# JackShDr/InfluentialRS

Measured on AMD Instinct MI355X. Metric: scored user-item pairs/sec (whole node), higher is better.
Workload: dtype f32; 1 GPU; c2: n_item=3415, d=128, L=200, H=4, layers=6, ffn=256; one greedy path-search step; users_per_gpu=4096, top_k=100, sweep=bf16 filter + exact f32 re-score, parallelism=single GPU

## Files before the change

### influentialrs_amd/csrc/irs_internal.h

```cpp
#pragma once

#include <hip/hip_runtime.h>
#include <stdint.h>
#include <stdio.h>
#include <string.h>

#include "../../include/irs_hip.h"

#if !defined(IRS_LAB) && (defined(X6_DUMP) || defined(X6_STAMP) || defined(X6_NO_SPLIT) || defined(X6_NO_MFMA) ||            \
                          defined(X6_NO_READS) || defined(X6_NO_DMA) || defined(X6_NO_BARRIER) || defined(X6_NO_QKV_STORE) ||  \
                          defined(X6_NW) || defined(SEQ_EXP) || defined(PLAN_STAMP) || defined(ATTN_STAMP) ||                  \
                          defined(IRS_SMALL_TIMING) || defined(IRS_DIRECT_TIMING))
#error "a lab switch (X6_* / SEQ_EXP / *_STAMP / IRS_*_TIMING) is defined without IRS_LAB: the product library must be built without them"
#endif

#include <atomic>
#include <functional>
#define IRS_MAX_DEVICES 32
static inline int irs_cur_dev() {
    int d = 0;
    if (hipGetDevice(&d) != hipSuccess || d < 0 || d >= IRS_MAX_DEVICES) d = 0;
    return d;
}
#define IRS_ONCE_PER_DEVICE(body_)                                                                                        \
    do {                                                                                                                  \
        static std::atomic<unsigned> once_mask_{0};                                                                       \
        const unsigned once_bit_ = 1u << irs_cur_dev();                                                                   \
        if (!(once_mask_.load(std::memory_order_acquire) & once_bit_)) {                                                  \
            body_;                                                                                                        \
            once_mask_.fetch_or(once_bit_, std::memory_order_release);                                                    \
        }                                                                                                                 \
    } while (0)

#define IRS_MAX_LAYERS 16
#define IRS_CAND_BUCKETS 64
#define IRS_CAND_SLOTS 64
#define IRS_CAND_CAP (IRS_CAND_BUCKETS * IRS_CAND_SLOTS)
#define IRS_REFINE_CAP 1024
#define IRS_MAX_GROUPS 2048
#define IRS_MAX_PATH 64
#define IRS_MAX_EXCL 4096
#define IRS_LSE_SLOTS_RING 4096
#define IRS_COOP_FALLBACK_MIN_ITEMS 262144
#define IRS_EXH_SCRATCH_KEYS (64 * 32768)

struct irs_layer_w {
    const float *sa_in_w, *sa_in_b, *sa_out_w, *sa_out_b;
    const float *ca_in_w, *ca_in_b, *ca_out_w, *ca_out_b;
    const float *l1_w, *l1_b, *l2_w, *l2_b;
    const float *n1_w, *n1_b, *n2_w, *n2_b, *n3_w, *n3_b;
};

struct irs_prof_ev {
    hipEvent_t a, b;
};

enum { IRS_STEP_GREEDY = 1, IRS_STEP_BEAM, IRS_STEP_SHARDED_BEAM, IRS_STEP_SHARDED_BEAM_SPLIT };
struct irs_step_key {
    int32_t kind, B, W, P, k, sweep, sample, sample_k;
    uint64_t seed;
    const void *comm, *seq, *user, *hep, *paths, *status;
    const void *tr_item, *tr_target, *tr_rank, *tr_scratch;
    int32_t arr_rank;
    uint32_t arr_lp_bits;
};
static_assert(sizeof(irs_step_key) == 8 * sizeof(int32_t) + 11 * 8 + 2 * sizeof(int32_t), "irs_step_key is compared with memcmp: no padding");
struct irs_step_graph {
    hipGraphExec_t exec;
    irs_step_key key;
};

struct irs_excl {
    const int64_t *rows;
    const int32_t *cnt;
    const int32_t *map;
    const float *paths;
    const int32_t *step_ptr;
    int stride, div;
    int path_ld, path_by_user;
    int step_arg, on;
};

struct irs_beam_state {
    int64_t *seq;
    int32_t *hep;
    double *cum;
    float *paths;
    int32_t *fin;
};
struct irs_beam_side {
    int64_t *user;
    int32_t *done;
    int32_t *map;
};
struct irs_beam_cand {
    const float *val;
// ... 591 lines not shown
```

### influentialrs_amd/csrc/score.hip

```cpp
#include <type_traits>

#include "irs_internal.h"

typedef __attribute__((ext_vector_type(16))) float f32x16;
typedef __attribute__((ext_vector_type(8))) __bf16 bf16x8;

#define MODE_PRE 0
#define MODE_EMIT 1
#define MODE_COUNT 2
#define MODE_DENSE 3
#define MODE_LSE 4
#define MODE_CEGRAD 5
#define MODE_TRACE 6

struct SweepArgs {
    const uint4 *wp;
    const float *w32;
    const float *bias;
    const uint4 *xb;
    const float *x32;
    int M, M_pad, UT, d;
    int64_t n_local;
    int tile_begin, tile_end, tiles_per_wave, n_strips, n_ublocks;
    int tile_stride;
// ... 1333 lines not shown
    int row = blockIdx.x * 4 + (threadIdx.x >> 6);
    int lane = threadIdx.x & 63;
    if (fb_count && blockIdx.x == 0 && threadIdx.x == 0) *fb_count = 0u;
    if (row >= M_pad) return;
    cand_cnt[(size_t)row * IRS_CAND_BUCKETS + lane] = 0u;
    if (lane == 0 && row < M) status[row] = 0;
    const int ut = row >> 5, r = row & 31;
    float ss = 0.f, ssr = 0.f, ssd = 0.f;
    if (lane < 2 * KS) {
        uint4 v = pack8_bf16(x + (size_t)row * d, 8 * lane, d, row < M, ss, ssr, ssd);
        xb[((size_t)ut * KS + (lane >> 1)) * 64 + (lane & 1) * 32 + r] = v;
    }
    ss = lanes_sum<63>(ss);
    ssr = lanes_sum<63>(ssr);
    ssd = lanes_sum<63>(ssd);
    if (lane == 0) {
        const float nx = sqrtf(fmaxf(ss, ssr)), ndx = sqrtf(ssd);
        const float e = (row < M) ? 1.001f * (ndx * wn[0] + nx * wn[1]) + acc_factor * (1.001f * nx * wn[0] + wn[2]) : 0.f;
        eps[row] = e;
        if (thr_carry && row < M) {
            float t = thr_carry[row];
            if (!(t == t)) t = -INFINITY, thr_carry[row] = t;
            traw_carry[row] = t > -INFINITY ? t + 2.0f * e : -INFINITY;
        }
    }
}

__global__ void k_zero_eps(float *eps, int n) {
    int i = blockIdx.x * blockDim.x + threadIdx.x;
    if (i < n) eps[i] = 0.f;
}

__global__ void __launch_bounds__(256) k_pack_w(const float *__restrict__ W, const float *__restrict__ b, int64_t n_local,
                                                int n_tiles, int d, int KS, uint4 *__restrict__ wp,
                                                float *__restrict__ bias_pad, unsigned int *__restrict__ wn_bits) {
    int64_t row = (int64_t)blockIdx.x * 4 + (threadIdx.x >> 6);
    int lane = threadIdx.x & 63;
    if (row >= (int64_t)n_tiles * 32) return;
    const int64_t t = row >> 5;
    const int r = (int)(row & 31);
    float ss = 0.f, ssr = 0.f, ssd = 0.f;
    if (lane < 2 * KS) {
        uint4 v = pack8_bf16(W + (size_t)row * d, 8 * lane, d, row < n_local, ss, ssr, ssd);
        wp[((size_t)t * KS + (lane >> 1)) * 64 + (lane & 1) * 32 + r] = v;
    }
    ss = lanes_sum<63>(ss);
    ssr = lanes_sum<63>(ssr);
    ssd = lanes_sum<63>(ssd);
    if (lane == 0) {
        bias_pad[row] = (row < n_local) ? b[row] : -INFINITY;
        if (row < n_local) {
            atomicMax(wn_bits + 0, __float_as_uint(sqrtf(fmaxf(ss, ssr)) * 1.001f));
            atomicMax(wn_bits + 1, __float_as_uint(sqrtf(ssd) * 1.001f));
            atomicMax(wn_bits + 2, __float_as_uint(fabsf(b[row])));
        }
    }
}

#define SEL2_G IRS_MAX_GROUPS
static_assert(SEL2_G == 2048, "k_select_thr_bits: 32 keys per lane");
template <int CTRL>
__device__ __forceinline__ unsigned int dpp_u32(unsigned int v) {
    return (unsigned int)__builtin_amdgcn_update_dpp(0, (int)v, CTRL, 0xF, 0xF, true);
}
__device__ __forceinline__ unsigned int wave_sum_u32(unsigned int v) {
    v += dpp_u32<0xB1>(v);
    v += dpp_u32<0x4E>(v);
    v += dpp_u32<0x141>(v);
    v += dpp_u32<0x140>(v);
    return (unsigned int)__builtin_amdgcn_readlane((int)v, 0) + (unsigned int)__builtin_amdgcn_readlane((int)v, 16) +
           (unsigned int)__builtin_amdgcn_readlane((int)v, 32) + (unsigned int)__builtin_amdgcn_readlane((int)v, 48);
}
__device__ __forceinline__ unsigned int wave_max_u32(unsigned int v) {
    unsigned int o;
    o = dpp_u32<0xB1>(v), v = o > v ? o : v;
    o = dpp_u32<0x4E>(v), v = o > v ? o : v;
    o = dpp_u32<0x141>(v), v = o > v ? o : v;
    o = dpp_u32<0x140>(v), v = o > v ? o : v;
    const unsigned int a = (unsigned int)__builtin_amdgcn_readlane((int)v, 0), b = (unsigned int)__builtin_amdgcn_readlane((int)v, 16);
    const unsigned int c = (unsigned int)__builtin_amdgcn_readlane((int)v, 32), d = (unsigned int)__builtin_amdgcn_readlane((int)v, 48);
    const unsigned int ab = a > b ? a : b, cd = c > d ? c : d;
    return ab > cd ? ab : cd;
}
__global__ void __launch_bounds__(256) k_select_thr_bits(const float *__restrict__ gm, int G, int M, int M_pad, int k,
                                                         const float *__restrict__ eps, float *__restrict__ thr,
                                                         float *__restrict__ traw) {
    constexpr int STRIDE = SEL2_G + 16;
    constexpr int KPL = SEL2_G / 64;
    __shared__ unsigned int sel_lds[4 * STRIDE];
    const int tid = threadIdx.x;
    {
        const int rl = tid & 3, tq = tid >> 2;
        const int row = blockIdx.x * 4 + rl;
        const float *blk = gm + (size_t)blockIdx.x * G * 4 + rl;
        float raw[KPL];
#pragma unroll
        for (int i = 0; i < KPL; ++i) {
            const int g = tq + 64 * i;
            raw[i] = blk[(size_t)(g < G ? g : G - 1) * 4];
        }
#pragma unroll
        for (int i = 0; i < KPL; ++i) asm volatile("" : "+v"(raw[i]));
#pragma unroll
        for (int i = 0; i < KPL; ++i) {
            const int g = tq + 64 * i;
            const unsigned int kk = irs_fkey(raw[i]);
            sel_lds[rl * STRIDE + g] = (g < G && row < M) ? kk : 0u;
        }
    }
    __syncthreads();
    const int lane = tid & 63;
    const int wave = __builtin_amdgcn_readfirstlane(tid >> 6);
    const int row = blockIdx.x * 4 + wave;
    unsigned int key[KPL];
    unsigned int mx = 0u, mnc = 0u;
#pragma unroll
    for (int i = 0; i < KPL; ++i) {
        key[i] = sel_lds[wave * STRIDE + lane + 64 * i];
        mx = key[i] > mx ? key[i] : mx;
        const unsigned int c = (lane + 64 * i < G) ? ~key[i] : 0u;
        mnc = c > mnc ? c : mnc;
    }
    const unsigned int smx = wave_max_u32(mx), smn = ~wave_max_u32(mnc);
    const unsigned int diff = smx ^ smn;
    const int top = diff ? 31 - __builtin_clz(diff) : -1;
    unsigned int prefix = top >= 31 ? 0u : (smx & ~((2u << top) - 1u));
    if (top < 0) prefix = smx;
    for (int bit = top; bit >= 0; --bit) {
        const unsigned int cand = prefix | (1u << bit);
        unsigned int c0 = 0, c1 = 0, c2 = 0, c3 = 0;
#pragma unroll
        for (int i = 0; i < KPL; i += 4) {
            c0 += key[i] >= cand ? 1u : 0u;
            c1 += key[i + 1] >= cand ? 1u : 0u;
            c2 += key[i + 2] >= cand ? 1u : 0u;
            c3 += key[i + 3] >= cand ? 1u : 0u;
        }
        const unsigned int cnt = wave_sum_u32((c0 + c1) + (c2 + c3));
        if (cnt >= (unsigned int)k) prefix = cand;
    }
    if (lane == 0 && row < M_pad) {
        const bool enough = G >= k;
        const float t = enough ? irs_unkey(prefix) : -INFINITY;
        thr[row] = (row < M) ? (enough ? t - 2.0f * eps[row] : -INFINITY) : INFINITY;
        traw[row] = (row < M) ? t : INFINITY;
    }
}

__device__ __forceinline__ void bitonic_desc(unsigned long long *keys, int n) {
    for (int size = 2; size <= n; size <<= 1) {
        for (int stride = size >> 1; stride > 0; stride >>= 1) {
            __syncthreads();
            for (int i = threadIdx.x; i < n / 2; i += blockDim.x) {
                int lo = 2 * i - (i & (stride - 1));
                int hi = lo + stride;
                bool desc = ((lo & size) == 0);
                unsigned long long a = keys[lo], b = keys[hi];
                if ((a < b) == desc) {
                    keys[lo] = b;
                    keys[hi] = a;
                }
            }
        }
    }
    __syncthreads();
}

__device__ __forceinline__ void radix_find_bin(const unsigned int *hist, unsigned int need, int lane, int shift,
                                               unsigned int *s_prefix, unsigned int *s_k) {
    const unsigned int h0 = hist[4 * lane], h1 = hist[4 * lane + 1], h2 = hist[4 * lane + 2], h3 = hist[4 * lane + 3];
    const unsigned int own = h0 + h1 + h2 + h3;
// ... 70 lines not shown
        if (i < (int)n) {
            unsigned long long kk = buf[i];
            val[(size_t)row * k + i] = irs_unkey((unsigned int)(kk >> 32));
            ids[(size_t)row * k + i] = item_lo + (int64_t)(0xFFFFFFFFu - (unsigned int)kk);
        } else {
            val[(size_t)row * k + i] = -INFINITY;
            ids[(size_t)row * k + i] = -1;
        }
    }
    if (tid == 0 && (int)n < k) status[row] |= IRS_ROW_FEWER_THAN_K;
}

#define EXH_FB_MAX 64
#define EXH_STRIPS 256
#define EXH_KEYS_PER_ROW 32768

template <typename KeyFn>
__device__ __forceinline__ unsigned int exh_select(KeyFn &&keyfn, int64_t j0, int64_t j1, int k, unsigned long long *buf) {
    __shared__ unsigned int s_n;
    __shared__ unsigned long long s_thr;
    const int tid = threadIdx.x;
    __syncthreads();
    if (tid == 0) {
        s_n = 0;
        s_thr = 0ull;
    }
    __syncthreads();
    for (int64_t base = j0; base < j1; base += 256) {
        const int64_t j = base + tid;
        if (j < j1) {
            const unsigned long long key = keyfn(j);
            if (key > s_thr) {
                const unsigned int slot = atomicAdd(&s_n, 1u);
                buf[slot] = key;
            }
        }
        __syncthreads();
        if (s_n > EXH_BUF - 256) {
            const unsigned int n = s_n;
            for (int i = n + tid; i < EXH_BUF; i += 256) buf[i] = 0ull;
            bitonic_desc(buf, EXH_BUF);
            if (tid == 0) {
                s_n = (n < (unsigned int)k) ? n : k;
                if (n >= (unsigned int)k) s_thr = buf[k - 1];
            }
            __syncthreads();
        }
    }
    const unsigned int n = s_n;
    for (int i = n + tid; i < EXH_BUF; i += 256) buf[i] = 0ull;
    bitonic_desc(buf, EXH_BUF);
    __syncthreads();
    return n < (unsigned int)k ? n : (unsigned int)k;
}

__global__ void __launch_bounds__(256) k_exh_strips(const float *__restrict__ x, int d, const float *__restrict__ W,
                                                    const float *__restrict__ bias, int64_t n_local, int k, int n_strips,
                                                    const unsigned int *__restrict__ fb_count, const int32_t *__restrict__ fb_list,
                                                    unsigned long long *__restrict__ exh_keys) {
    __shared__ unsigned long long buf[EXH_BUF];
    __shared__ float xs[256];
    unsigned int nfb = *fb_count;
    if (nfb == 0u) return;
    if (nfb > EXH_FB_MAX) nfb = EXH_FB_MAX;
    const int strip = blockIdx.x;
    const int64_t per = (n_local + n_strips - 1) / n_strips;
    const int64_t j0 = (int64_t)strip * per, j1 = (j0 + per < n_local) ? j0 + per : n_local;
    for (unsigned int fi = blockIdx.y; fi < nfb; fi += gridDim.y) {
        const int row = fb_list[fi];
        __syncthreads();
        for (int i = threadIdx.x; i < d; i += 256) xs[i] = x[(size_t)row * d + i];
        __syncthreads();
        const unsigned int n = exh_select(
            [&](int64_t j) -> unsigned long long {
                const float e = irs_chain(xs, W + (size_t)j * d, bias[j], d);
                return ((unsigned long long)irs_fkey(e) << 32) | (0xFFFFFFFFu - (unsigned int)j);
            },
            j0, j1, k, buf);
        unsigned long long *o = exh_keys + ((size_t)fi * n_strips + strip) * k;
        for (int i = threadIdx.x; i < k; i += 256) o[i] = i < (int)n ? buf[i] : 0ull;
    }
}

__global__ void __launch_bounds__(256) k_refine(const float *__restrict__ x, int d, const float *__restrict__ W,
                                                const float *__restrict__ bias, const unsigned int *__restrict__ cnt,
                                                const unsigned long long *__restrict__ cand,
                                                const float *__restrict__ eps, const float *__restrict__ traw, int k,
                                                int64_t item_lo, int64_t n_local, float *__restrict__ val,
                                                int64_t *__restrict__ ids, int32_t *__restrict__ status,
                                                unsigned int *__restrict__ fb_count, int32_t *__restrict__ fb_list) {
    __shared__ __attribute__((aligned(16))) unsigned long long ckeys[IRS_CAND_CAP + 2];
    unsigned long long *rkeys = ckeys;
    __shared__ unsigned int hist[256];
    __shared__ float xs[256];
    __shared__ unsigned int boff[IRS_CAND_BUCKETS + 1];
    __shared__ unsigned int s_prefix, s_k, s_nr, s_above, s_over;
    const int row = blockIdx.x, tid = threadIdx.x;
    constexpr int PER = IRS_CAND_BUCKETS * IRS_CAND_SLOTS / 256;
    unsigned long long cv[PER];
#pragma unroll
    for (int j = 0; j < PER; ++j) {
        const int idx = tid + 256 * j;
        cv[j] = cand[((size_t)row * IRS_CAND_BUCKETS + idx / IRS_CAND_SLOTS) * IRS_CAND_SLOTS + idx % IRS_CAND_SLOTS];
    }
    for (int i = tid; i < d; i += 256) xs[i] = x[(size_t)row * d + i];
    if (tid < IRS_CAND_BUCKETS) hist[tid] = cnt[(size_t)row * IRS_CAND_BUCKETS + tid];
    __syncthreads();
    if (tid < 64) {
        const unsigned int cb = hist[tid] & ~IRS_CAND_OVERFLOW;
        const unsigned int cl = cb > IRS_CAND_SLOTS ? IRS_CAND_SLOTS : cb;
        unsigned int incl = cl;
#pragma unroll
        for (int o = 1; o < 64; o <<= 1) {
            const unsigned int t = __shfl_up(incl, o, 64);
            if (tid >= o) incl += t;
        }
        boff[tid] = incl - cl;
        if (tid == 63) boff[IRS_CAND_BUCKETS] = incl;
        const unsigned long long ov = __ballot((hist[tid] & IRS_CAND_OVERFLOW) != 0u);
        if (tid == 0) {
            s_over = ov ? 1u : 0u;
            s_prefix = 0;
            s_k = k;
            s_nr = 0;
            s_above = 0;
        }
    }
    __syncthreads();
    if (s_over) {
        if (tid == 0) status[row] |= IRS_ROW_FALLBACK;
        if (fb_count) {
            if (tid == 0) fb_list[atomicAdd(fb_count, 1u)] = row;
            return;
        }
        exhaustive_row(x, d, W, bias, n_local, item_lo, k, row, val, ids, status, ckeys, xs, true);
        return;
    }
    const unsigned int c = boff[IRS_CAND_BUCKETS];
#pragma unroll
    for (int j = 0; j < PER; ++j) {
        const int idx = tid + 256 * j;
        const int b = idx / IRS_CAND_SLOTS, sl = idx % IRS_CAND_SLOTS;
        if ((unsigned int)sl < boff[b + 1] - boff[b]) ckeys[boff[b] + sl] = cv[j];
    }
    __syncthreads();
    const float t1 = traw[row];
    if (t1 > -INFINITY) {
        unsigned int mine = 0;
        for (int i = tid; i < (int)c; i += 256) mine += (irs_unkey((unsigned int)(ckeys[i] >> 32)) >= t1) ? 1u : 0u;
        if (mine) atomicAdd(&s_above, mine);
        __syncthreads();
        if (s_above < (unsigned int)k) {
            if (tid == 0) status[row] |= IRS_ROW_FALLBACK;
            if (fb_count) {
                if (tid == 0) fb_list[atomicAdd(fb_count, 1u)] = row;
                return;
            }
            exhaustive_row(x, d, W, bias, n_local, item_lo, k, row, val, ids, status, ckeys, xs, false);
            return;
        }
    }
    float thr2 = -INFINITY;
    if (c >= (unsigned int)k) {
        for (int pass = 0; pass < 4; ++pass) {
            const int shift = 24 - 8 * pass;
            hist[tid] = 0;
            __syncthreads();
            const unsigned int prefix = s_prefix;
            for (int i0 = 0; i0 < (int)c; i0 += 256) {
                const int i = i0 + tid;
                const unsigned int key = i < (int)c ? (unsigned int)(ckeys[i] >> 32) : 0u;
                const bool match = i < (int)c && ((pass == 0) || ((key >> (shift + 8)) == (prefix >> (shift + 8))));
                const unsigned int bin = (key >> shift) & 255;
                const unsigned long long m = __ballot(match);
                if (m) {
                    const unsigned int first = __builtin_amdgcn_readlane(bin, __builtin_ctzll(m));
                    if (__ballot(match && bin == first) == m) {
                        if ((tid & 63) == __builtin_ctzll(m)) atomicAdd(&hist[first], (unsigned int)__popcll(m));
                    } else if (match)
                        atomicAdd(&hist[bin], 1u);
                }
            }
            __syncthreads();
            if (tid < 64) radix_find_bin(hist, s_k, tid, shift, &s_prefix, &s_k);
            __syncthreads();
        }
        thr2 = irs_unkey(s_prefix) - 2.0f * eps[row];
    }
    {
        constexpr int PERC = IRS_CAND_CAP / 256;
        unsigned int keep[PERC];
#pragma unroll
        for (int j = 0; j < PERC; ++j) {
            const int i = tid + 256 * j;
            keep[j] = 0xFFFFFFFFu;
            if (i < (int)c) {
                const unsigned long long key = ckeys[i];
                if (irs_unkey((unsigned int)(key >> 32)) >= thr2) keep[j] = (unsigned int)key;
            }
        }
        __syncthreads();
#pragma unroll
        for (int j = 0; j < PERC; ++j)
            if (keep[j] != 0xFFFFFFFFu) rkeys[atomicAdd(&s_nr, 1u)] = (unsigned long long)keep[j];
    }
    __syncthreads();
    const unsigned int nr = s_nr;
    for (int i = tid; i < (int)nr; i += 256) {
        unsigned int j = (unsigned int)rkeys[i];
        float e = irs_chain(xs, W + (size_t)j * d, bias[j], d);
        rkeys[i] = ((unsigned long long)irs_fkey(e) << 32) | (0xFFFFFFFFu - j);
    }
    if ((nr & 1) && tid == 0) rkeys[nr] = 0ull;
    __syncthreads();
    {
        const ulonglong2 *r2 = reinterpret_cast<const ulonglong2 *>(rkeys);
        for (int i = tid; i < (int)nr; i += 256) {
            const unsigned long long me = rkeys[i];
            int above = 0;
            for (int j = 0; j < (int)(nr + 1) / 2; ++j) {
                const ulonglong2 v = r2[j];
                above += (v.x > me) + (v.y > me);
            }
            if (above < k) {
                val[(size_t)row * k + above] = irs_unkey((unsigned int)(me >> 32));
                ids[(size_t)row * k + above] = item_lo + (int64_t)(0xFFFFFFFFu - (unsigned int)me);
            }
        }
        for (int i = (int)nr + tid; i < k; i += 256) {
            val[(size_t)row * k + i] = -INFINITY;
            ids[(size_t)row * k + i] = -1;
        }
    }
    if (tid == 0 && (int)nr < k) status[row] |= IRS_ROW_FEWER_THAN_K;
}

#define DIRECT_MAX_ITEMS 4096
#define DIRECT_TILE 64
#define DIRECT_MAX_D 256
#ifdef IRS_DIRECT_TIMING
__device__ unsigned long long g_direct_t[16];
#define DSTAMP(i) do { if (threadIdx.x == 0) tstamp[i] = __builtin_amdgcn_s_memtime(); } while (0)
#else
#define DSTAMP(i)
#endif
#define DIRECT_ROWS 8
template <int MODE, int SLOTS = IRS_WIN_SLOTS_SHORT>
__global__ void __launch_bounds__(256) k_topk_direct(const float *__restrict__ x, int d, const float *__restrict__ W,
                                                     const float *__restrict__ bias, int n_local, int64_t item_lo, int k,
                                                     unsigned long long *__restrict__ gkeys, unsigned int *__restrict__ arrive,
                                                     float *__restrict__ val, int64_t *__restrict__ ids,
                                                     int32_t *__restrict__ status, irs_path_args pa, int M) {
    __shared__ __attribute__((aligned(16))) float tile[DIRECT_TILE * (DIRECT_MAX_D + 4)];
    __shared__ __attribute__((aligned(16))) unsigned long long rkeys[IRS_REFINE_CAP + 2];
    __shared__ __attribute__((aligned(16))) float xs[(MODE == 1 ? DIRECT_ROWS : 1) * DIRECT_MAX_D];
    __shared__ __attribute__((aligned(16))) unsigned long long tmax[256];
    __shared__ unsigned int wsum[4];
    __shared__ unsigned int s_last, s_thr;
    const int row = MODE == 1 ? blockIdx.y * DIRECT_ROWS : blockIdx.y, tid = threadIdx.x, lane = tid & 63, wave = tid >> 6;
#ifdef IRS_DIRECT_TIMING
    unsigned long long tstamp[10];
#endif
    DSTAMP(0);
    unsigned int *gk = reinterpret_cast<unsigned int *>(gkeys + (size_t)row * IRS_CAND_CAP);
    if constexpr (MODE != 2) {
    const bool vec = (d & 3) == 0;
    const int S = vec ? ((d & 7) ? d : d + 4) : (d | 1);
    const int j0 = blockIdx.x * DIRECT_TILE;
    const int nj = min(DIRECT_TILE, n_local - j0);
    const int d4 = d >> 2;
    if (vec) {
        for (int i = tid; i < nj * d4; i += 256) {
            const int jj = i / d4, c4 = i - jj * d4;
            *reinterpret_cast<float4 *>(tile + jj * S + 4 * c4) = reinterpret_cast<const float4 *>(W + (size_t)j0 * d)[i];
        }
    } else {
        for (int i = tid; i < nj * d; i += 256) {
            const int jj = i / d, c = i - jj * d;
            tile[jj * S + c] = W[(size_t)j0 * d + i];
        }
    }
    if constexpr (MODE == 1) {
        for (int i = tid; i < DIRECT_ROWS * d; i += 256) {
            const int rr = i / d, c = i - rr * d;
            xs[rr * DIRECT_MAX_D + c] = (row + rr < M) ? x[(size_t)(row + rr) * d + c] : 0.f;
        }
        __syncthreads();
        if (lane < nj) {
            const float b0 = bias[j0 + lane];
            float acc0 = b0, acc1 = b0;
            const float *x0 = xs + wave * DIRECT_MAX_D, *x1 = xs + (wave + 4) * DIRECT_MAX_D;
            if (vec) {
                const float4 *w4 = reinterpret_cast<const float4 *>(tile + lane * S);
                for (int c = 0; c < d4; ++c) {
                    const float4 wv = w4[c], xa = reinterpret_cast<const float4 *>(x0)[c], xb = reinterpret_cast<const float4 *>(x1)[c];
                    acc0 = __fmaf_rn(xa.x, wv.x, acc0), acc1 = __fmaf_rn(xb.x, wv.x, acc1);
                    acc0 = __fmaf_rn(xa.y, wv.y, acc0), acc1 = __fmaf_rn(xb.y, wv.y, acc1);
                    acc0 = __fmaf_rn(xa.z, wv.z, acc0), acc1 = __fmaf_rn(xb.z, wv.z, acc1);
                    acc0 = __fmaf_rn(xa.w, wv.w, acc0), acc1 = __fmaf_rn(xb.w, wv.w, acc1);
                }
            } else {
                const float *wr = tile + lane * S;
                for (int c = 0; c < d; ++c) acc0 = __fmaf_rn(x0[c], wr[c], acc0), acc1 = __fmaf_rn(x1[c], wr[c], acc1);
            }
            if (row + wave < M) gk[(size_t)wave * (IRS_CAND_CAP * 2) + j0 + lane] = irs_fkey(acc0);
            if (row + wave + 4 < M) gk[(size_t)(wave + 4) * (IRS_CAND_CAP * 2) + j0 + lane] = irs_fkey(acc1);
        }
        return;
    }
    for (int i = tid; i < d; i += 256) xs[i] = x[(size_t)row * d + i];
    __syncthreads();
    DSTAMP(1);
    if (wave == 0 && lane < nj) {
        float acc = bias[j0 + lane];
        if (vec) {
            const float4 *w4 = reinterpret_cast<const float4 *>(tile + lane * S);
            const float4 *x4 = reinterpret_cast<const float4 *>(xs);
// ... 434 lines not shown
    sweep_decompose(a, 0, ctx->n_tiles, 1, tpw);
    *slots = a.n_strips * 4 * 2;
    if (*slots > 2 * max_waves) IRS_FAIL(ctx, IRS_E_UNSUPPORTED, "lse slots %d > %d", *slots, 2 * max_waves);
    a.lse_part = ctx->lse_part;
    return IRS_OK;
}

static void sweep_f32_whole(const irs_ctx *ctx, SweepArgs &a, const float *xrows, int M) {
    sweep_common(ctx, a, xrows, M);
    const int nub = (a.UT + ub_f32(ctx->KS) - 1) / ub_f32(ctx->KS);
    sweep_decompose(a, 0, ctx->n_tiles, nub, 0);
}

template <bool EMIT>
static int launch_lse_f32(irs_ctx *ctx, SweepArgs &a, hipStream_t s) {
    const int KS = ctx->KS;
    if (lse_ring_ok(ctx, a)) {
        a.n_ublocks = 1;
        constexpr int SPW = LSE_RING_NW / 4;
        const int nwg = (a.n_strips + SPW - 1) / SPW;
        dim3 grid(((nwg + 7) / 8) * 8);
        const size_t lds = (size_t)LSE_RING_NW * LSE_RING_WAVE_B + (size_t)LSE_RING_NW * (EMIT_Q * 12 + 16);
        IRS_ONCE_PER_DEVICE({
            (void)hipFuncSetAttribute(reinterpret_cast<const void *>(k_lse_ring<16, EMIT, LSE_RING_NW, LSE_RING_CK>), hipFuncAttributeMaxDynamicSharedMemorySize, (int)lds);
            (void)hipFuncSetAttribute(reinterpret_cast<const void *>(k_lse_ring<8, EMIT, LSE_RING_NW, LSE_RING_CK>), hipFuncAttributeMaxDynamicSharedMemorySize, (int)lds);
        });
        if (KS == 16) hipLaunchKernelGGL((k_lse_ring<16, EMIT, LSE_RING_NW, LSE_RING_CK>), grid, dim3(64 * LSE_RING_NW), lds, s, a);
        else hipLaunchKernelGGL((k_lse_ring<8, EMIT, LSE_RING_NW, LSE_RING_CK>), grid, dim3(64 * LSE_RING_NW), lds, s, a);
        IRS_CHECK_HIP(ctx, hipGetLastError());
        return IRS_OK;
    }
    const bool xreg = a.UT == 1 && KS == 16;
    const int UB = xreg ? 1 : ub_f32(KS);
    a.n_ublocks = (a.UT + UB - 1) / UB;
    dim3 grid(((a.n_strips + 7) / 8) * 8 * a.n_ublocks);
    const size_t lds = (size_t)UB * KS * 2048 + EMIT_Q_BYTES;
#define L_(KS_, UB_, XR_)                                                                                                 \
    do {                                                                                                                  \
        IRS_ONCE_PER_DEVICE((void)hipFuncSetAttribute(reinterpret_cast<const void *>(k_lse_f32<KS_, UB_, EMIT, XR_>),     \
                                                      hipFuncAttributeMaxDynamicSharedMemorySize, (int)lds));             \
        hipLaunchKernelGGL((k_lse_f32<KS_, UB_, EMIT, XR_>), grid, dim3(256), lds, s, a);                                 \
    } while (0)
    switch (KS) {
    case 2: L_(2, 8, false); break;
    case 4: L_(4, 8, false); break;
    case 8: L_(8, 4, false); break;
    case 16: if (xreg) L_(16, 1, true); else L_(16, 2, false); break;
    default: IRS_FAIL(ctx, IRS_E_UNSUPPORTED, "unsupported d_pad %d", ctx->d_pad);
    }
#undef L_
    IRS_CHECK_HIP(ctx, hipGetLastError());
    return IRS_OK;
}

int irs_launch_pack_w(irs_ctx *ctx, hipStream_t s) {
    IRS_CHECK_HIP(ctx, hipMemsetAsync(ctx->wnorm_max, 0, 4 * sizeof(float), s));
    int64_t rows = (int64_t)ctx->n_tiles * 32;
    hipLaunchKernelGGL(k_pack_w, dim3((unsigned)((rows + 3) / 4)), dim3(256), 0, s, ctx->proj_w, ctx->proj_b,
                       ctx->n_local, ctx->n_tiles, ctx->dims.d, ctx->KS, ctx->wp,
                       ctx->bias_pad, reinterpret_cast<unsigned int *>(ctx->wnorm_max));
    IRS_CHECK_HIP(ctx, hipGetLastError());
    return IRS_OK;
}

bool irs_topk_is_direct(const irs_ctx *ctx, int M, int k) {
    return M <= 1024 && ctx->n_local <= DIRECT_MAX_ITEMS && k <= 256 && ctx->dims.d <= DIRECT_MAX_D;
}

enum TopkForm {
    TOPK_DIRECT1,
    TOPK_DIRECT2,
    TOPK_SWEPT,
};
struct TopkPlan {
    TopkForm form;
    bool fused_lse;
    bool lse_after;
    bool reuse_thr;
    bool coop_fb;
    int stride;
    int nt0;
    int tpw0;
    int r_sel;
};

static TopkPlan topk_plan(const irs_ctx *ctx, const float *xrows, int M, int k, int sweep, bool want_lse, int carry) {
    TopkPlan p{};
    if (irs_topk_is_direct(ctx, M, k)) {
        p.form = M <= 32 ? TOPK_DIRECT1 : TOPK_DIRECT2;
        p.lse_after = want_lse;
        return p;
    }
    p.form = TOPK_SWEPT;
    SweepArgs a;
    sweep_common(ctx, a, xrows, M);
    p.fused_lse = want_lse && sweep == IRS_SWEEP_BF16 && lse_fast_ok(ctx, a);
    p.lse_after = want_lse && !p.fused_lse;
    p.coop_fb = ctx->n_local >= IRS_COOP_FALLBACK_MIN_ITEMS && ctx->exh_keys != nullptr;
    const int nt = ctx->n_tiles;
    p.reuse_thr = carry && ctx->carry_period > 0 && sweep == IRS_SWEEP_BF16 && !p.fused_lse && ctx->thr_valid && ctx->thr_M == M &&
                  ctx->thr_k == k && ctx->thr_age + 1 < ctx->carry_period && nt >= 2 * 8 * 1024;
    if (p.reuse_thr) return p;
    int nt0 = nt >= 16 * 1024 ? nt / 16 : nt / 8;
    if (nt0 < 1024) nt0 = 1024;
    if (nt0 > nt) nt0 = nt;
    p.stride = nt / nt0;
    p.nt0 = (nt + p.stride - 1) / p.stride;
    p.tpw0 = (p.nt0 + 1023) / 1024;
    p.r_sel = k;
    if (p.stride > 1) {
        p.r_sel = ((p.stride >= 16 ? 4 : 3) * k + p.stride - 1) / p.stride;
        if (p.r_sel < 8) p.r_sel = 8;
        if (p.r_sel > k) p.r_sel = k;
    }
    return p;
}

static int topk_direct(irs_ctx *ctx, const TopkPlan &p, const float *xrows, int M, int k, float *val, int64_t *ids0,
                       int32_t *status, const irs_path_args *path, hipStream_t s) {
    irs_prof_begin(ctx, IRS_PROF_REFINE, s);
    const unsigned int tiles = (unsigned)((ctx->n_local + DIRECT_TILE - 1) / DIRECT_TILE);
    unsigned int *arrive = reinterpret_cast<unsigned int *>(ctx->step_ctr) + 8;
    const irs_path_args pa = path ? *path : irs_path_args{};
    constexpr int S16 = IRS_WIN_SLOTS_LONG;
    const bool long_win = path && irs_window_slots(ctx) == S16;
    if (p.form == TOPK_DIRECT1)
        hipLaunchKernelGGL((long_win ? k_topk_direct<0, S16> : k_topk_direct<0>), dim3(tiles, M), dim3(256), 0, s, xrows, ctx->dims.d, ctx->proj_w, ctx->proj_b,
                           (int)ctx->n_local, ctx->shard.item_lo, k, ctx->cand, arrive, val, ids0, status, pa, M);
    else {
        hipLaunchKernelGGL(k_topk_direct<1>, dim3(tiles, (M + DIRECT_ROWS - 1) / DIRECT_ROWS), dim3(256), 0, s, xrows, ctx->dims.d,
                           ctx->proj_w, ctx->proj_b, (int)ctx->n_local, ctx->shard.item_lo, k, ctx->cand, arrive, val, ids0,
                           status, irs_path_args{}, M);
        hipLaunchKernelGGL((long_win ? k_topk_direct<2, S16> : k_topk_direct<2>), dim3(1, M), dim3(256), 0, s, xrows, ctx->dims.d, ctx->proj_w, ctx->proj_b,
                           (int)ctx->n_local, ctx->shard.item_lo, k, ctx->cand, arrive, val, ids0, status, pa, M);
    }
    irs_prof_end(ctx, IRS_PROF_REFINE, s, 2.0 * ctx->dims.d * (double)M * (double)ctx->n_local, 0.0);
    IRS_CHECK_HIP(ctx, hipGetLastError());
    return IRS_OK;
}

static int topk_prep(irs_ctx *ctx, const TopkPlan &p, const float *xrows, int M, int M_pad, int sweep, int32_t *status,
                     hipStream_t s) {
    static_assert(IRS_CAND_BUCKETS == 64, "k_prep_x resets one bucket counter per lane");
    if (sweep == IRS_SWEEP_BF16) {
        const float acc_factor = (float)(ctx->d_pad + 8) * 2.384185791015625e-07f;
        hipLaunchKernelGGL(k_prep_x, dim3((M_pad + 3) / 4), dim3(256), 0, s, xrows, M, M_pad, ctx->dims.d, ctx->KS,
                           ctx->xb, ctx->eps, ctx->wnorm_max, acc_factor, ctx->cand_cnt, status, p.coop_fb ? ctx->fb_count : nullptr,
                           p.reuse_thr ? ctx->thr : nullptr, p.reuse_thr ? ctx->ref_tmp : nullptr);
    } else {
        IRS_CHECK_HIP(ctx, hipMemsetAsync(status, 0, sizeof(int32_t) * M, s));
        IRS_CHECK_HIP(ctx, hipMemsetAsync(ctx->cand_cnt, 0, sizeof(unsigned int) * (size_t)M_pad * IRS_CAND_BUCKETS, s));
        hipLaunchKernelGGL(k_zero_eps, dim3((M_pad + 255) / 256), dim3(256), 0, s, ctx->eps, M_pad);
    }
    IRS_CHECK_HIP(ctx, hipGetLastError());
    return IRS_OK;
}

static int topk_select(irs_ctx *ctx, const TopkPlan &p, SweepArgs &a, int M, int sweep, hipStream_t s) {
    sweep_decompose(a, 0, ctx->n_tiles, 1, p.tpw0, p.stride);
    const int G = 2 * a.n_strips * 4;
    if (G > SEL2_G) IRS_FAIL(ctx, IRS_E_UNSUPPORTED, "pre-pass groups %d > %d", G, SEL2_G);
    a.gm = ctx->gm;
    a.n_groups = G;
    irs_prof_begin(ctx, IRS_PROF_SWEEP, s);
    const int rc = sweep == IRS_SWEEP_BF16 ? launch_sweep_bf16<MODE_PRE>(ctx, a, s) : launch_sweep_f32<MODE_PRE>(ctx, a, s);
    irs_prof_end(ctx, IRS_PROF_SWEEP, s, 2.0 * ctx->dims.d * (double)M * p.nt0 * 32.0,
                 (double)p.nt0 * 32.0 * ctx->d_pad * (sweep == IRS_SWEEP_BF16 ? 2.0 : 4.0));
    if (rc) return rc;
    hipLaunchKernelGGL(k_select_thr_bits, dim3((a.M_pad + 3) / 4), dim3(256), 0, s, ctx->gm, G, M, a.M_pad, p.r_sel, ctx->eps,
                       ctx->thr, ctx->ref_tmp);
    IRS_CHECK_HIP(ctx, hipGetLastError());
    return IRS_OK;
}

static int topk_emit(irs_ctx *ctx, const TopkPlan &p, SweepArgs &a, int M, int sweep, float *lse_max, float *lse_sum,
                     hipStream_t s) {
    a.thr = ctx->thr;
    a.cnt = ctx->cand_cnt;
    a.cand = ctx->cand;
    int lse_slots = 0, rc;
    if (p.fused_lse) {
        if ((rc = lse_decompose(ctx, a, &lse_slots))) return rc;
    } else {
        const int UB = sweep == IRS_SWEEP_BF16 ? ub_bf16(ctx->KS) : ub_f32(ctx->KS);
        sweep_decompose(a, 0, ctx->n_tiles, (a.UT + UB - 1) / UB, 0);
    }
    const double flops = 2.0 * ctx->dims.d * (double)M * (double)ctx->n_local;
    const double bytes = (double)ctx->n_tiles * 32.0 * ctx->d_pad * ((sweep == IRS_SWEEP_BF16 && !p.fused_lse) ? 2.0 : 4.0);
    irs_prof_begin(ctx, IRS_PROF_SWEEP, s);
    irs_prof_begin(ctx, IRS_PROF_SWEEP_EMIT, s);
    if (p.fused_lse) rc = launch_lse_f32<true>(ctx, a, s);
    else if (sweep == IRS_SWEEP_BF16) rc = launch_sweep_bf16<MODE_EMIT>(ctx, a, s);
    else rc = launch_sweep_f32<MODE_EMIT>(ctx, a, s);
    irs_prof_end(ctx, IRS_PROF_SWEEP, s, flops, bytes);
    irs_prof_end(ctx, IRS_PROF_SWEEP_EMIT, s, flops, bytes);
    if (rc) return rc;
    if (p.fused_lse) {
        hipLaunchKernelGGL(k_lse_reduce, dim3(M), dim3(256), 0, s, ctx->lse_part, lse_slots, a.M_pad, M, lse_max, lse_sum);
        IRS_CHECK_HIP(ctx, hipGetLastError());
    }
    return IRS_OK;
}

static int topk_refine(irs_ctx *ctx, const TopkPlan &p, const float *xrows, int M, int k, int sweep, float *val, int64_t *ids0,
                       int32_t *status, hipStream_t s) {
    const int d = ctx->dims.d;
    irs_prof_begin(ctx, IRS_PROF_REFINE, s);
    if (p.coop_fb && sweep != IRS_SWEEP_BF16) IRS_CHECK_HIP(ctx, hipMemsetAsync(ctx->fb_count, 0, sizeof(unsigned int), s));
    hipLaunchKernelGGL(k_refine, dim3(M), dim3(256), 0, s, xrows, d, ctx->proj_w, ctx->proj_b, ctx->cand_cnt, ctx->cand,
                       ctx->eps, ctx->ref_tmp, k, ctx->shard.item_lo, ctx->n_local, val, ids0, status,
                       p.coop_fb ? ctx->fb_count : nullptr, ctx->fb_list);
    if (p.coop_fb) {
        int ns = EXH_STRIPS;
        while (ns > 1 && (long long)ns * k > EXH_KEYS_PER_ROW) ns >>= 1;
        hipLaunchKernelGGL(k_exh_strips, dim3(ns, 4), dim3(256), 0, s, xrows, d, ctx->proj_w, ctx->proj_b, ctx->n_local, k, ns,
                           ctx->fb_count, ctx->fb_list, ctx->exh_keys);
        hipLaunchKernelGGL(k_exh_merge, dim3(EXH_FB_MAX), dim3(256), 0, s, xrows, d, ctx->proj_w, ctx->proj_b, ctx->n_local,
                           ctx->shard.item_lo, k, ns, ctx->fb_count, ctx->fb_list, ctx->exh_keys, val, ids0, status);
    }
    irs_prof_end(ctx, IRS_PROF_REFINE, s, 0.0, 0.0);
    IRS_CHECK_HIP(ctx, hipGetLastError());
    return IRS_OK;
}

int irs_launch_topk(irs_ctx *ctx, const float *xrows, int M, int k, int sweep, float *val, int64_t *ids0,
                    int32_t *status, hipStream_t s, const irs_path_args *path, float *lse_max, float *lse_sum, int carry) {
    const TopkPlan p = topk_plan(ctx, xrows, M, k, sweep, lse_max != nullptr, carry);
    if (path && p.form == TOPK_SWEPT) IRS_FAIL(ctx, IRS_E_STATE, "fused path step needs the direct top-k");
    int rc;
    if (p.form != TOPK_SWEPT) {
        if ((rc = topk_direct(ctx, p, xrows, M, k, val, ids0, status, path, s))) return rc;
    } else {
        SweepArgs a;
        sweep_common(ctx, a, xrows, M);
        if ((rc = topk_prep(ctx, p, xrows, M, a.M_pad, sweep, status, s))) return rc;
        if (p.reuse_thr) ++ctx->thr_age;
        else {
            if ((rc = topk_select(ctx, p, a, M, sweep, s))) return rc;
            ctx->thr_valid = sweep == IRS_SWEEP_BF16, ctx->thr_M = M, ctx->thr_k = k, ctx->thr_age = 0;
        }
        if ((rc = topk_emit(ctx, p, a, M, sweep, lse_max, lse_sum, s))) return rc;
        if ((rc = topk_refine(ctx, p, xrows, M, k, sweep, val, ids0, status, s))) return rc;
    }
    return p.lse_after ? irs_launch_lse(ctx, xrows, M, lse_max, lse_sum, s) : IRS_OK;
}

int irs_launch_topk_exhaustive(irs_ctx *ctx, const float *xrows, int M, int k, float *val, int64_t *ids0,
                               int32_t *status, hipStream_t s) {
    IRS_CHECK_HIP(ctx, hipMemsetAsync(status, 0, sizeof(int32_t) * M, s));
    hipLaunchKernelGGL(k_exhaustive, dim3(M), dim3(256), 0, s, xrows, ctx->dims.d, ctx->proj_w, ctx->proj_b,
                       ctx->n_local, ctx->shard.item_lo, k, 0, val, ids0, status);
    IRS_CHECK_HIP(ctx, hipGetLastError());
    return IRS_OK;
}

int irs_launch_gather(irs_ctx *ctx, const float *xrows, int M, const int64_t *ids0, int g, float *out, hipStream_t s) {
    hipLaunchKernelGGL(k_gather, dim3(M), dim3(64), 0, s, xrows, ctx->dims.d, ctx->proj_w, ctx->proj_b,
                       ctx->shard.item_lo, ctx->n_local, ids0, g, out);
    IRS_CHECK_HIP(ctx, hipGetLastError());
    return IRS_OK;
}

int irs_launch_count_before(irs_ctx *ctx, const float *xrows, int M, const float *ref_score, const int64_t *ref_id0,
                            const int64_t *excl, int n_excl, int64_t *count, hipStream_t s) {
    SweepArgs a;
    sweep_f32_whole(ctx, a, xrows, M);
    IRS_CHECK_HIP(ctx, hipMemsetAsync(count, 0, sizeof(int64_t) * M, s));
    int64_t *ref_local = reinterpret_cast<int64_t *>(ctx->cand);
    hipLaunchKernelGGL(k_localize_ref, dim3((M + 255) / 256), dim3(256), 0, s, ref_id0, ctx->shard.item_lo, ref_local, M);
    a.ref_score = ref_score;
    a.ref_id = ref_local;
    a.count = reinterpret_cast<unsigned long long *>(count);
    irs_prof_begin(ctx, IRS_PROF_SWEEP, s);
    int rc = launch_sweep_f32<MODE_COUNT>(ctx, a, s);
    irs_prof_end(ctx, IRS_PROF_SWEEP, s, 2.0 * ctx->dims.d * (double)M * (double)ctx->n_local,
                 (double)ctx->n_local * ctx->dims.d * 4.0);
    if (rc) return rc;
    if (excl && n_excl > 0) {
        hipLaunchKernelGGL(k_count_excl, dim3(M), dim3(64), 0, s, xrows, ctx->dims.d, ctx->proj_w, ctx->proj_b,
                           ctx->shard.item_lo, ctx->n_local, ref_score, ref_id0, excl, n_excl,
                           reinterpret_cast<unsigned long long *>(count));
    }
    IRS_CHECK_HIP(ctx, hipGetLastError());
    return IRS_OK;
}

int irs_launch_dense(irs_ctx *ctx, const float *xrows, int M, float *out, int64_t ld, hipStream_t s) {
    SweepArgs a;
    sweep_f32_whole(ctx, a, xrows, M);
    a.dense = out;
    a.ld = ld;
    irs_prof_begin(ctx, IRS_PROF_SWEEP, s);
// ... 196 lines not shown
```

Before: 2.394 billion pairs/s.

## Add sparse refine path skipping radix select for small candidate sets; template threshold select

Adds a SPARSE variant of the refine kernel that loads only the occupied candidate slots per bucket via wave-level readlane, computes the bucket prefix in registers instead of through LDS with an extra barrier, and uses a wave-reduced count. When the candidate count is at most 512, it skips the four-pass radix threshold select and re-scores all candidates exactly. The threshold-select kernel is also templated on keys per lane so small group counts use a smaller register and LDS footprint. The trade-off is that small-candidate rows now do more exact f32 dot products in place of the radix passes. Lab-only timestamp instrumentation is added behind a compile switch.

```diff
diff --git a/influentialrs_amd/csrc/irs_internal.h b/influentialrs_amd/csrc/irs_internal.h
--- a/influentialrs_amd/csrc/irs_internal.h
+++ b/influentialrs_amd/csrc/irs_internal.h
@@ -10,8 +10,8 @@
 #if !defined(IRS_LAB) && (defined(X6_DUMP) || defined(X6_STAMP) || defined(X6_NO_SPLIT) || defined(X6_NO_MFMA) ||            \
                           defined(X6_NO_READS) || defined(X6_NO_DMA) || defined(X6_NO_BARRIER) || defined(X6_NO_QKV_STORE) ||  \
                           defined(X6_NW) || defined(SEQ_EXP) || defined(PLAN_STAMP) || defined(ATTN_STAMP) ||                  \
-                          defined(IRS_SMALL_TIMING) || defined(IRS_DIRECT_TIMING))
-#error "a lab switch (X6_* / SEQ_EXP / *_STAMP / IRS_*_TIMING) is defined without IRS_LAB: the product library must be built without them"
+                          defined(IRS_SMALL_TIMING) || defined(IRS_DIRECT_TIMING) || defined(REFINE_STAMP) || defined(REFINE_ALL_MAX))
+#error "a lab switch (X6_* / SEQ_EXP / *_STAMP / IRS_*_TIMING / REFINE_ALL_MAX) is defined without IRS_LAB: the product library must be built without them"
 #endif
 
 #include <atomic>
diff --git a/influentialrs_amd/csrc/score.hip b/influentialrs_amd/csrc/score.hip
--- a/influentialrs_amd/csrc/score.hip
+++ b/influentialrs_amd/csrc/score.hip
@@ -1439,11 +1439,12 @@
     const unsigned int ab = a > b ? a : b, cd = c > d ? c : d;
     return ab > cd ? ab : cd;
 }
+template <int KPL>
 __global__ void __launch_bounds__(256) k_select_thr_bits(const float *__restrict__ gm, int G, int M, int M_pad, int k,
                                                          const float *__restrict__ eps, float *__restrict__ thr,
                                                          float *__restrict__ traw) {
-    constexpr int STRIDE = SEL2_G + 16;
-    constexpr int KPL = SEL2_G / 64;
+    static_assert(KPL % 4 == 0 && 64 * KPL <= SEL2_G, "four partial counts per bit; at most SEL2_G keys per row");
+    constexpr int STRIDE = 64 * KPL + 16;
     __shared__ unsigned int sel_lds[4 * STRIDE];
     const int tid = threadIdx.x;
     {
@@ -1680,6 +1681,27 @@
     }
 }
 
+#ifdef REFINE_ALL_MAX
+#define IRS_REFINE_ALL_MAX REFINE_ALL_MAX
+#else
+#define IRS_REFINE_ALL_MAX 512
+#endif
+#ifdef REFINE_STAMP
+#define REFINE_STAMP_ROWS 8192
+__device__ unsigned long long g_refine_t[8 * REFINE_STAMP_ROWS];
+extern "C" void *irs_lab_refine_stamps() {
+    void *p = nullptr;
+    return hipGetSymbolAddress(&p, HIP_SYMBOL(g_refine_t)) == hipSuccess ? p : nullptr;
+}
+#define RSTAMP_BEGIN unsigned long long rstamp[8] = {__builtin_amdgcn_s_memtime()}
+#define RSTAMP(i) rstamp[i] = __builtin_amdgcn_s_memtime()
+#define RSTAMP_END do { if (threadIdx.x == 0 && blockIdx.x < REFINE_STAMP_ROWS) for (int i_ = 0; i_ < 8; ++i_) g_refine_t[8 * blockIdx.x + i_] = rstamp[i_]; } while (0)
+#else
+#define RSTAMP_BEGIN
+#define RSTAMP(i)
+#define RSTAMP_END
+#endif
+template <bool SPARSE>
 __global__ void __launch_bounds__(256) k_refine(const float *__restrict__ x, int d, const float *__restrict__ W,
                                                 const float *__restrict__ bias, const unsigned int *__restrict__ cnt,
                                                 const unsigned long long *__restrict__ cand,
@@ -1694,59 +1716,117 @@
     __shared__ unsigned int boff[IRS_CAND_BUCKETS + 1];
     __shared__ unsigned int s_prefix, s_k, s_nr, s_above, s_over;
     const int row = blockIdx.x, tid = threadIdx.x;
+    RSTAMP_BEGIN;
     constexpr int PER = IRS_CAND_BUCKETS * IRS_CAND_SLOTS / 256;
     unsigned long long cv[PER];
-#pragma unroll
-    for (int j = 0; j < PER; ++j) {
-        const int idx = tid + 256 * j;
-        cv[j] = cand[((size_t)row * IRS_CAND_BUCKETS + idx / IRS_CAND_SLOTS) * IRS_CAND_SLOTS + idx % IRS_CAND_SLOTS];
-    }
-    for (int i = tid; i < d; i += 256) xs[i] = x[(size_t)row * d + i];
-    if (tid < IRS_CAND_BUCKETS) hist[tid] = cnt[(size_t)row * IRS_CAND_BUCKETS + tid];
-    __syncthreads();
-    if (tid < 64) {
-        const unsigned int cb = hist[tid] & ~IRS_CAND_OVERFLOW;
+    unsigned int c;
+    float t1s = 0.f, e1s = 0.f;
+    if constexpr (SPARSE) {
+        static_assert(IRS_CAND_BUCKETS == 64 && IRS_CAND_SLOTS == 64, "one lane per bucket, one lane per slot");
+        const int lane = tid & 63;
+        const int wave = __builtin_amdgcn_readfirstlane(tid >> 6);
+        const unsigned int raw = cnt[(size_t)row * IRS_CAND_BUCKETS + lane];
+        t1s = traw[row];
+        e1s = eps[row];
+        for (int i = tid; i < d; i += 256) xs[i] = x[(size_t)row * d + i];
+        const unsigned int cb = raw & ~IRS_CAND_OVERFLOW;
         const unsigned int cl = cb > IRS_CAND_SLOTS ? IRS_CAND_SLOTS : cb;
         unsigned int incl = cl;
 #pragma unroll
         for (int o = 1; o < 64; o <<= 1) {
             const unsigned int t = __shfl_up(incl, o, 64);
-            if (tid >= o) incl += t;
-        }
-        boff[tid] = incl - cl;
-        if (tid == 63) boff[IRS_CAND_BUCKETS] = incl;
-        const unsigned long long ov = __ballot((hist[tid] & IRS_CAND_OVERFLOW) != 0u);
+            if (lane >= o) incl += t;
+        }
+        const unsigned int excl = incl - cl;
+        if (__ballot((raw & IRS_CAND_OVERFLOW) != 0u)) {
+            if (tid == 0) status[row] |= IRS_ROW_FALLBACK;
+            if (fb_count) {
+                if (tid == 0) fb_list[atomicAdd(fb_count, 1u)] = row;
+                return;
+            }
+            exhaustive_row(x, d, W, bias, n_local, item_lo, k, row, val, ids, status, ckeys, xs, true);
+            return;
+        }
+        c = (unsigned int)__builtin_amdgcn_readlane((int)incl, 63);
+        const unsigned long long *rc = cand + (size_t)row * IRS_CAND_CAP;
+#pragma unroll
+        for (int j = 0; j < PER; ++j) {
+            const int b = wave + 4 * j;
+            const unsigned int n = (unsigned int)__builtin_amdgcn_readlane((int)cl, b);
+            cv[j] = rc[(unsigned int)lane < n ? b * IRS_CAND_SLOTS + lane : 0];
+        }
+#pragma unroll
+        for (int j = 0; j < PER; ++j) {
+            const int b = wave + 4 * j;
+            const unsigned int n = (unsigned int)__builtin_amdgcn_readlane((int)cl, b);
+            const unsigned int o = (unsigned int)__builtin_amdgcn_readlane((int)excl, b);
+            if ((unsigned int)lane < n) ckeys[o + lane] = cv[j];
+        }
         if (tid == 0) {
-            s_over = ov ? 1u : 0u;
             s_prefix = 0;
             s_k = k;
             s_nr = 0;
             s_above = 0;
         }
-    }
-    __syncthreads();
-    if (s_over) {
-        if (tid == 0) status[row] |= IRS_ROW_FALLBACK;
-        if (fb_count) {
-            if (tid == 0) fb_list[atomicAdd(fb_count, 1u)] = row;
+        __syncthreads();
+    } else {
+#pragma unroll
+        for (int j = 0; j < PER; ++j) {
+            const int idx = tid + 256 * j;
+            cv[j] = cand[((size_t)row * IRS_CAND_BUCKETS + idx / IRS_CAND_SLOTS) * IRS_CAND_SLOTS + idx % IRS_CAND_SLOTS];
+        }
+        for (int i = tid; i < d; i += 256) xs[i] = x[(size_t)row * d + i];
+        if (tid < IRS_CAND_BUCKETS) hist[tid] = cnt[(size_t)row * IRS_CAND_BUCKETS + tid];
+        __syncthreads();
+        if (tid < 64) {
+            const unsigned int cb = hist[tid] & ~IRS_CAND_OVERFLOW;
+            const unsigned int cl = cb > IRS_CAND_SLOTS ? IRS_CAND_SLOTS : cb;
+            unsigned int incl = cl;
+#pragma unroll
+            for (int o = 1; o < 64; o <<= 1) {
+                const unsigned int t = __shfl_up(incl, o, 64);
+                if (tid >= o) incl += t;
+            }
+            boff[tid] = incl - cl;
+            if (tid == 63) boff[IRS_CAND_BUCKETS] = incl;
+            const unsigned long long ov = __ballot((hist[tid] & IRS_CAND_OVERFLOW) != 0u);
+            if (tid == 0) {
+                s_over = ov ? 1u : 0u;
+                s_prefix = 0;
+                s_k = k;
+                s_nr = 0;
+                s_above = 0;
+            }
+        }
+        __syncthreads();
+        if (s_over) {
+            if (tid == 0) status[row] |= IRS_ROW_FALLBACK;
+            if (fb_count) {
+                if (tid == 0) fb_list[atomicAdd(fb_count, 1u)] = row;
+                return;
+            }
+            exhaustive_row(x, d, W, bias, n_local, item_lo, k, row, val, ids, status, ckeys, xs, true);
             return;
         }
-        exhaustive_row(x, d, W, bias, n_local, item_lo, k, row, val, ids, status, ckeys, xs, true);
-        return;
-    }
-    const unsigned int c = boff[IRS_CAND_BUCKETS];
-#pragma unroll
-    for (int j = 0; j < PER; ++j) {
-        const int idx = tid + 256 * j;
-        const int b = idx / IRS_CAND_SLOTS, sl = idx % IRS_CAND_SLOTS;
-        if ((unsigned int)sl < boff[b + 1] - boff[b]) ckeys[boff[b] + sl] = cv[j];
-    }
-    __syncthreads();
-    const float t1 = traw[row];
+        c = boff[IRS_CAND_BUCKETS];
+#pragma unroll
+        for (int j = 0; j < PER; ++j) {
+            const int idx = tid + 256 * j;
+            const int b = idx / IRS_CAND_SLOTS, sl = idx % IRS_CAND_SLOTS;
+            if ((unsigned int)sl < boff[b + 1] - boff[b]) ckeys[boff[b] + sl] = cv[j];
+        }
+        __syncthreads();
+    }
+    RSTAMP(1);
+    const float t1 = SPARSE ? t1s : traw[row];
     if (t1 > -INFINITY) {
         unsigned int mine = 0;
         for (int i = tid; i < (int)c; i += 256) mine += (irs_unkey((unsigned int)(ckeys[i] >> 32)) >= t1) ? 1u : 0u;
-        if (mine) atomicAdd(&s_above, mine);
+        if constexpr (SPARSE) {
+            const unsigned int mine_w = wave_sum_u32(mine);
+            if ((tid & 63) == 0 && mine_w) atomicAdd(&s_above, mine_w);
+        } else if (mine)
+            atomicAdd(&s_above, mine);
         __syncthreads();
         if (s_above < (unsigned int)k) {
             if (tid == 0) status[row] |= IRS_ROW_FALLBACK;
@@ -1758,8 +1838,10 @@
             return;
         }
     }
+    RSTAMP(2);
+    const bool all = SPARSE && IRS_REFINE_ALL_MAX > 0 && c <= (unsigned int)IRS_REFINE_ALL_MAX && t1 > -INFINITY;
     float thr2 = -INFINITY;
-    if (c >= (unsigned int)k) {
+    if (!all && c >= (unsigned int)k) {
         for (int pass = 0; pass < 4; ++pass) {
             const int shift = 24 - 8 * pass;
             hist[tid] = 0;
@@ -1783,9 +1865,10 @@
             if (tid < 64) radix_find_bin(hist, s_k, tid, shift, &s_prefix, &s_k);
             __syncthreads();
         }
-        thr2 = irs_unkey(s_prefix) - 2.0f * eps[row];
-    }
-    {
+        thr2 = irs_unkey(s_prefix) - 2.0f * (SPARSE ? e1s : eps[row]);
+    }
+    RSTAMP(3);
+    if (!all) {
         constexpr int PERC = IRS_CAND_CAP / 256;
         unsigned int keep[PERC];
 #pragma unroll
@@ -1795,6 +1878,7 @@
             if (i < (int)c) {
                 const unsigned long long key = ckeys[i];
                 if (irs_unkey((unsigned int)(key >> 32)) >= thr2) keep[j] = (unsigned int)key;
+                if (SPARSE && (int64_t)(unsigned int)key >= n_local) keep[j] = 0xFFFFFFFFu;
             }
         }
         __syncthreads();
@@ -1803,7 +1887,8 @@
             if (keep[j] != 0xFFFFFFFFu) rkeys[atomicAdd(&s_nr, 1u)] = (unsigned long long)keep[j];
     }
     __syncthreads();
-    const unsigned int nr = s_nr;
+    const unsigned int nr = all ? c : s_nr;
+    RSTAMP(4);
     for (int i = tid; i < (int)nr; i += 256) {
         unsigned int j = (unsigned int)rkeys[i];
         float e = irs_chain(xs, W + (size_t)j * d, bias[j], d);
@@ -1811,6 +1896,7 @@
     }
     if ((nr & 1) && tid == 0) rkeys[nr] = 0ull;
     __syncthreads();
+    RSTAMP(5);
     {
         const ulonglong2 *r2 = reinterpret_cast<const ulonglong2 *>(rkeys);
         for (int i = tid; i < (int)nr; i += 256) {
@@ -1831,6 +1917,8 @@
         }
     }
     if (tid == 0 && (int)nr < k) status[row] |= IRS_ROW_FEWER_THAN_K;
+    RSTAMP(6);
+    RSTAMP_END;
 }
 
 #define DIRECT_MAX_ITEMS 4096
@@ -2431,6 +2519,7 @@
     int nt0;
     int tpw0;
     int r_sel;
+    bool refine_sparse;
 };
 
 static TopkPlan topk_plan(const irs_ctx *ctx, const float *xrows, int M, int k, int sweep, bool want_lse, int carry) {
@@ -2457,6 +2546,7 @@
     p.nt0 = (nt + p.stride - 1) / p.stride;
     p.tpw0 = (p.nt0 + 1023) / 1024;
     p.r_sel = k;
+    p.refine_sparse = p.stride == 1;
     if (p.stride > 1) {
         p.r_sel = ((p.stride >= 16 ? 4 : 3) * k + p.stride - 1) / p.stride;
         if (p.r_sel < 8) p.r_sel = 8;
@@ -2516,8 +2606,8 @@
     irs_prof_end(ctx, IRS_PROF_SWEEP, s, 2.0 * ctx->dims.d * (double)M * p.nt0 * 32.0,
                  (double)p.nt0 * 32.0 * ctx->d_pad * (sweep == IRS_SWEEP_BF16 ? 2.0 : 4.0));
     if (rc) return rc;
-    hipLaunchKernelGGL(k_select_thr_bits, dim3((a.M_pad + 3) / 4), dim3(256), 0, s, ctx->gm, G, M, a.M_pad, p.r_sel, ctx->eps,
-                       ctx->thr, ctx->ref_tmp);
+    hipLaunchKernelGGL((G <= 256 ? k_select_thr_bits<4> : k_select_thr_bits<SEL2_G / 64>), dim3((a.M_pad + 3) / 4), dim3(256), 0, s,
+                       ctx->gm, G, M, a.M_pad, p.r_sel, ctx->eps, ctx->thr, ctx->ref_tmp);
     IRS_CHECK_HIP(ctx, hipGetLastError());
     return IRS_OK;
 }
@@ -2556,7 +2646,7 @@
     const int d = ctx->dims.d;
     irs_prof_begin(ctx, IRS_PROF_REFINE, s);
     if (p.coop_fb && sweep != IRS_SWEEP_BF16) IRS_CHECK_HIP(ctx, hipMemsetAsync(ctx->fb_count, 0, sizeof(unsigned int), s));
-    hipLaunchKernelGGL(k_refine, dim3(M), dim3(256), 0, s, xrows, d, ctx->proj_w, ctx->proj_b, ctx->cand_cnt, ctx->cand,
+    hipLaunchKernelGGL((p.refine_sparse ? k_refine<true> : k_refine<false>), dim3(M), dim3(256), 0, s, xrows, d, ctx->proj_w, ctx->proj_b, ctx->cand_cnt, ctx->cand,
                        ctx->eps, ctx->ref_tmp, k, ctx->shard.item_lo, ctx->n_local, val, ids0, status,
                        p.coop_fb ? ctx->fb_count : nullptr, ctx->fb_list);
     if (p.coop_fb) {
```

Measured after the change: 2.409 billion pairs/s, median of 6. About the same (+0.6%).
